# pnkraemer/experiments-lanczos-adjoints

Measured on AMD Instinct MI355X. Metric: slq_logdet_value_and_grad_throughput, higher is better.
Workload: dtype f32 (Gram contraction emulated with 3 f16 MFMA products, fp32 accumulate; accuracy vs fp64 at this size on 32 probe sets, profiles/r05b_accuracy_16_seeds/: value <= 5.6e-6 and d/d raw_noise <= 1.3e-5 on all 32; the other two gradient components <= 1e-4 on 25 of 32 sets, <= 1.5e-4 on 29, worst 3.96e-; 1 GPU; matrix-free RBF GP kernel N=131072 d=8, SLQ log-det value+grad, 40 Lanczos steps (full reortho) x 64 probes, fp32 (BASELINE config 4); N=131072, d=8, krylov_depth=40, probes_total=64, probes_on_this_rank=64, rows_on_this_rank=131072, gram_precision=f16x3, kernel=rbf

## Files before the change

experiments-lanczos-adjoints_amd/csrc/mfx_rbf.h:

```cpp
#pragma once
#include <type_traits>

#include "mfx_internal.h"

namespace mfx {

constexpr int kRbfMaxD = 1024;
inline int rbf_dpad(int d) { return d <= 4 ? 4 : d <= 8 ? 8 : d <= 12 ? 12 : d <= 16 ? 16 : d <= kRbfMaxD ? (d + 31) / 32 * 32 : -1; }

template <int V>
using Const = std::integral_constant<int, V>;

template <typename Narrow, typename WideFn>
static void with_dpad(int dpad, Narrow&& narrow, WideFn&& wide) {
  switch (dpad) {
    case 4: narrow(Const<4>{}); break;
    case 8: narrow(Const<8>{}); break;
    case 12: narrow(Const<12>{}); break;
    case 16: narrow(Const<16>{}); break;
    case 32: narrow(Const<32>{}); break;
    default: wide(); break;
  }
}

template <int MAXD, typename Launch>
static int with_mfma_dpad(int dpad, const char* not_built, Launch&& launch) {
  int rc = MFX_ERR_UNSUPPORTED;
  auto arm = [&](auto dc) {
    if constexpr (decltype(dc)::value <= MAXD) rc = launch(dc);
    else set_error("%s", not_built);
  };
  with_dpad(dpad, arm, [&] {
    if (dpad == 64) arm(Const<64>{});
    else if (dpad == 96) arm(Const<96>{});
    else if (dpad == 128) arm(Const<128>{});
    else set_error("%s", not_built);
  });
  return rc;
}

template <typename F>
static auto with_bool(bool flag, F&& f) {
  return flag ? f(std::true_type{}) : f(std::false_type{});
}
template <typename F>
static int with_kind(int kernel_fn, F&& f) {
  switch (kernel_fn) {
    case MFX_KERNEL_RBF: return f(Const<MFX_KERNEL_RBF>{});
    case MFX_KERNEL_MATERN12: return f(Const<MFX_KERNEL_MATERN12>{});
    case MFX_KERNEL_MATERN32: return f(Const<MFX_KERNEL_MATERN32>{});
    case MFX_KERNEL_MATERN52: return f(Const<MFX_KERNEL_MATERN52>{});
    default: set_error("unknown kernel_fn %d", kernel_fn); return MFX_ERR_INVALID;
  }
}

inline bool vec4_ok(const void* a, int64_t lda, const void* b, int64_t ldb, int64_t n, int64_t nrow) {
  return (n % 4 == 0) && (nrow % 4 == 0) && (lda % 4 == 0) && (ldb % 4 == 0) && (reinterpret_cast<uintptr_t>(a) % 16 == 0) &&
         (reinterpret_cast<uintptr_t>(b) % 16 == 0);
}

enum class RbfApplyPath { valu, exact, h3 };
enum class RbfGradPath { valu, exact, split };
RbfApplyPath rbf_apply_path(const mfx_operator* op, int64_t p);
RbfGradPath rbf_grad_path(const mfx_operator* op, int64_t batch, bool have_hws);

constexpr int64_t kRbfVscaleFloats = 65536 * 3;
constexpr int64_t kRbfVscaleMaxP = (kRbfVscaleFloats - 64) / 4;
static_assert(kRbfVscaleMaxP == 49136, "the limit the error message of the split matvec states");
struct RbfVscaleLayout {
  int64_t scales, amax_bits, rangeflag, amax_part;
  int64_t gx;
  bool ok;
};
RbfVscaleLayout rbf_vscale_layout(int64_t n, int64_t p);

struct RbfPackLayout {
  int64_t P, chunks, ntile;
  int64_t off_a, off_part;
  int nsplit;
  int64_t ldpart, bytes;
};
RbfPackLayout rbf_pack_layout(int64_t n, int64_t nrow, int64_t p, int dpad);
int64_t rbf_pack_ws_bytes(const mfx_operator* op, int64_t p);

struct RbfGradHLayout {
  int64_t bpad, npad, npad_l;
  int64_t amaxL, amaxR, scl, tail, perm, Lh, Ll, Rh, Rl, bytes;
};
RbfGradHLayout rbf_grad_h_layout(int64_t n, int64_t nrow, int64_t batch);
inline int64_t rbf_grad_h_ws_bytes(int64_t n, int64_t batch) { return rbf_grad_h_layout(n, n, batch).bytes; }

int64_t rbf_mfma_grad_partial_rows(int64_t n);

int rbf_mfma_apply(const mfx_operator* op, const float* xs, const float* sq, int dpad, const float* x, int64_t ldx,
                   float* y, int64_t ldy, int64_t p, hipStream_t stream);
int rbf_mfma_apply_h3(const mfx_operator* op, const float* xs, const float* sq, int dpad, const float* x, int64_t ldx,
                      float* y, int64_t ldy, int64_t p, float* vscale, void* pk, hipStream_t stream);
int rbf_mfma_grad(const mfx_operator* op, const float* xs, const float* sq, int dpad, const float* L, int64_t ldl,
                  const float* R, int64_t ldr, int64_t batch, double* partial, int64_t* nblocks_out,
                  hipStream_t stream);
int rbf_mfma_grad_h(const mfx_operator* op, const float* xs, const float* sq, int dpad, const float* L, int64_t ldl,
                    const float* R, int64_t ldr, int64_t batch, int64_t inner, double* partial, int64_t* nblocks_out, void* hws,
                    const float** scales_out, hipStream_t stream);

struct RbfMatvecArgs {
  const float *xs, *sq;
  int64_t n;
  const float *outputscale, *noise, *vscale, *x;
  int64_t ldx;
  float* y;
  int64_t ldy, p;
  const void *pkv, *pka;
  float* part;
  const int* rangeflag;
  int64_t ldpart, row0, rend;
};
int rbf_fat_launch(int dpad, int nb, bool vec4, dim3 grid, hipStream_t stream, const RbfMatvecArgs& a);

}
```

experiments-lanczos-adjoints_amd/csrc/mfx_rbf_fat.hip:

```cpp
#include <type_traits>

#include "mfx_internal.h"
#include "mfx_rbf_common.h"

namespace mfx {

struct FatSplit {
  int e[16], h[8], m[16];
};
constexpr FatSplit kFatSplit2 = {{0, 1, 2, 3, 4, 5, 5, 6, 7, 8, 9, 10, 10, 11, 12, 13},
                                 {2, 4, 6, 7, 9, 11, 12, 14},
                                 {3, 4, 5, 6, 7, 8, 8, 9, 10, 11, 12, 13, 13, 14, 15, 16}};
constexpr FatSplit kFatSplit1 = {{0, 0, 1, 1, 2, 2, 3, 3, 4, 4, 5, 5, 6, 6, 7, 7},
                                 {1, 2, 3, 4, 5, 6, 7, 8},
                                 {2, 3, 3, 4, 4, 5, 5, 6, 6, 7, 7, 8, 8, 9, 9, 10}};
template <int NB, int NKD>
struct FatPlan;
template <>
struct FatPlan<2, 2> {
  static constexpr int kSlots = 14;
  static constexpr FatSplit kSplit = kFatSplit2;
  static constexpr int dist_q(int slot) { return slot == 10 ? 0 : (slot == 12 ? 1 : -1); }
  static constexpr int contr_m(int slot) { return slot < 10 ? slot : (slot == 11 ? 10 : (slot == 13 ? 11 : -1)); }
  static constexpr int slot_of(int m) { return m < 10 ? m : (m == 10 ? 11 : 13); }
// ... 166 lines not shown
      }
    }
  };
  auto split_slot = [&](const int slot, const int lag, floatx16& w, half8 (&ah)[2], half8 (&al)[2], unsigned (&lopk)[8], const bool neg) {
#pragma unroll
    for (int i = 0; i < 16; ++i)
      if (Plan::kSplit.e[i] == slot + kSlots * lag) split_op(w, ah, al, lopk, 0, i, neg);
#pragma unroll
    for (int i = 0; i < 8; ++i)
      if (Plan::kSplit.h[i] == slot + kSlots * lag) split_op(w, ah, al, lopk, 1, i, neg);
#pragma unroll
    for (int i = 0; i < 16; ++i)
      if (Plan::kSplit.m[i] == slot + kSlots * lag) split_op(w, ah, al, lopk, 2, i, neg);
  };

  __builtin_amdgcn_s_waitcnt(0x0F70);
  __builtin_amdgcn_s_barrier();
  asm volatile("" ::: "memory");

  constexpr bool kRing4 = NB == 1;
  floatx16 wr[kRing4 ? 4 : 3];
#define MFX_WC(blk) wr[kRing4 ? ((blk) & 3) : 0]
#define MFX_WN(blk) wr[kRing4 ? (((blk) + 1) & 3) : 1]
#define MFX_WD(blk) wr[kRing4 ? (((blk) + 2) & 3) : 2]
  half8 ahc[2], alc[2], ahn[2], aln[2];
  unsigned lpc[8], lpn[8];
  half8 vf[2][NB][2];
  half8 ajs[2][NKD];
  read_a(ajs[0], 0, 0);
#pragma unroll
  for (int s = 0; s < 2; ++s)
#pragma unroll
    for (int nb = 0; nb < NB; ++nb)
#pragma unroll
      for (int hl = 0; hl < 2; ++hl) read_v1(vf[s][nb][hl], 0, 0, s, nb, hl);
#pragma unroll
  for (int q = 0; q < NKD; ++q) dist_step(MFX_WC(0), ajs[0][q], bih[0][q], q == 0);
#pragma unroll
  for (int q = 0; q < NKD; ++q) dist_step(MFX_WN(0), ajs[0][q], bih[1][q], q == 0);
  asm volatile("" : "+v"(MFX_WC(0)));
#pragma unroll
  for (int slot = 0; slot < kSlots; ++slot) split_slot(slot, 0, MFX_WC(0), ahc, alc, lpc, false);

  const float sc = outputscale[0];
  int tl = 0;
  for (; tl < ntl; ++tl) {
    const int buf = tl & 1;
    if (tl > 0 && (tl % kChainTiles) == 0) {
#pragma unroll
      for (int mi = 0; mi < 4; ++mi)
#pragma unroll
        for (int nb = 0; nb < NB; ++nb)
#pragma unroll
          for (int r = 0; r < 16; ++r) {
            mst[mi][nb][r] += acc[mi][nb][r];
            acc[mi][nb][r] = 0.f;
          }
    }
#pragma unroll
    for (int blk = 0; blk < 8; ++blk) {
      const int jb = blk >> 2, mi = blk & 3;
      const int blk1 = (blk + 1) & 7, blk2 = (blk + 2) & 7;
      const int jb2 = blk2 >> 2, mi2 = blk2 & 3;
      const bool neg_c = ((jb + mi) & 1) != 0, neg_n = (((blk1 >> 2) + (blk1 & 3)) & 1) != 0;
      if (blk == 5 && tl + 2 < ntl) issue_tile_dma(tl + 2);
#pragma unroll
      for (int slot = 0; slot < kSlots; ++slot) {
        __builtin_amdgcn_sched_barrier(0);
        if (Plan::dist_q(slot) >= 0) {
          const int q = Plan::dist_q(slot);
          dist_step(MFX_WD(blk), ajs[jb2 & 1][q], bih[mi2][q], q == 0);
        } else {
          const int m = Plan::contr_m(slot);
          const int s = m / (3 * NB), nb = (m / 3) % NB, w = m % 3;
          acc[mi][nb] = __builtin_amdgcn_mfma_f32_32x32x16_f16(w == 2 ? alc[s] : ahc[s], w == 1 ? vf[s][nb][1] : vf[s][nb][0],
                                                               acc[mi][nb], 0, 0, 0);
        }
        __builtin_amdgcn_sched_barrier(0);
        split_slot(slot, 1, MFX_WC(blk), ahc, alc, lpc, neg_c);
        split_slot(slot, 0, MFX_WN(blk), ahn, aln, lpn, neg_n);
        if (mi == 1 && slot < NKD) {
          ajs[(jb + 1) & 1][slot] = *reinterpret_cast<const half8*>(reinterpret_cast<const _Float16*>(fat_smem + (jb == 1 ? buf ^ 1 : buf) * S::kTile) +
                                                                   (((jb + 1) & 1) * 32 + l31) * AROW + slot * 16 + lhi * 8);
        }
        if (mi == 3) {
#pragma unroll
          for (int s = 0; s < 2; ++s)
#pragma unroll
            for (int nb = 0; nb < NB; ++nb)
#pragma unroll
              for (int hl = 0; hl < 2; ++hl) {
                const int mlast = 3 * NB * s + 3 * nb + (hl ? 1 : 2);
                if (Plan::slot_of(mlast) == slot) read_v1(vf[s][nb][hl], jb == 1 ? buf ^ 1 : buf, (jb + 1) & 1, s, nb, hl);
              }
        }
      }
      __builtin_amdgcn_sched_barrier(0);
      if (blk == 4) {
        __builtin_amdgcn_s_waitcnt(0x0F70);
        __builtin_amdgcn_s_barrier();
        asm volatile("" ::: "memory");
      }
      ahc[0] = ahn[0]; ahc[1] = ahn[1];
      alc[0] = aln[0]; alc[1] = aln[1];
      if constexpr (!kRing4) {
        wr[0] = wr[1];
        wr[1] = wr[2];
      }
#pragma unroll
      for (int q = 0; q < 8; ++q) lpc[q] = lpn[q];
    }
  }
  __builtin_amdgcn_s_waitcnt(0x0F70);
#pragma unroll
  for (int mi = 0; mi < 4; ++mi)
#pragma unroll
    for (int nb = 0; nb < NB; ++nb)
#pragma unroll
      for (int r = 0; r < 16; ++r) acc[mi][nb][r] += mst[mi][nb][r];
  const float nz = gridDim.z > 1 ? 0.f : noise[0];
  float* yout = gridDim.z > 1 ? part + (int64_t)blockIdx.z * p * ldpart : y;
  const int64_t ldo = gridDim.z > 1 ? ldpart : ldy;
#pragma unroll
  for (int mi = 0; mi < 4; ++mi)
#pragma unroll
    for (int nb = 0; nb < NB; ++nb) {
      const int64_t b = b0 + nb * 32 + l31;
      if (b >= p) continue;
      const float sb = sc * vscale[2 * b + 1] * (1.f / 32768.f);
#pragma unroll
      for (int g = 0; g < 4; ++g) {
        const int64_t i = i_wave + mi * 32 + 8 * g + 4 * lhi;
        if (VEC4 && i + 3 < rend) {
          const float4 xv = *reinterpret_cast<const float4*>(x + b * ldx + i);
          float4 o;
          o.x = fmaf(sb, acc[mi][nb][4 * g + 0], nz * xv.x);
          o.y = fmaf(sb, acc[mi][nb][4 * g + 1], nz * xv.y);
          o.z = fmaf(sb, acc[mi][nb][4 * g + 2], nz * xv.z);
          o.w = fmaf(sb, acc[mi][nb][4 * g + 3], nz * xv.w);
          *reinterpret_cast<float4*>(yout + b * ldo + (i - row0)) = o;
        } else {
#pragma unroll
          for (int e = 0; e < 4; ++e)
            if (i + e < rend) yout[b * ldo + (i - row0) + e] = fmaf(sb, acc[mi][nb][4 * g + e], nz * x[b * ldx + i + e]);
        }
      }
    }
}

#undef MFX_WC
#undef MFX_WN
#undef MFX_WD

int rbf_fat_launch(int dpad, int nb, bool vec4, dim3 grid, hipStream_t stream, const RbfMatvecArgs& a) {
  const char* not_built = "fat-wave Gram matvec supports d <= 16 and chunks of 32 or 64 vectors";
  MFX_REQUIRE(nb == 1 || nb == 2, MFX_ERR_UNSUPPORTED, "%s", not_built);
  return with_mfma_dpad<16>(dpad, not_built, [&](auto dc) -> int {
    return with_bool(nb == 2, [&](auto two) -> int {
      return with_bool(vec4, [&](auto v4) -> int {
        constexpr int DPAD = decltype(dc)::value, NB = decltype(two)::value ? 2 : 1;
        k_rbf_fat_apply<DPAD, decltype(v4)::value, NB><<<grid, 256, FatSmem<DPAD, NB>::kTotal, stream>>>(
            a.xs, a.sq, a.n, a.outputscale, a.noise, a.vscale, a.x, a.ldx, a.y, a.ldy, a.p, static_cast<const uintx4*>(a.pkv),
            static_cast<const uintx4*>(a.pka), a.part, a.rangeflag, a.ldpart, a.row0, a.rend);
        MFX_CHECK_LAUNCH();
        return MFX_OK;
      });
    });
  });
}

}
```

experiments-lanczos-adjoints_amd/csrc/mfx_rbf_mfma.hip:

```cpp
#include <stdlib.h>

#include <type_traits>

#include "mfx_internal.h"
#include "mfx_rbf_common.h"

namespace mfx {

constexpr int kGM = 128, kGN = 128, kGK = 32, kGSplit = 8;
constexpr int kGSub = 8;
constexpr int kGLd = kGM + 4;


__device__ __forceinline__ float dist_factor(int kind) {
  return kind == MFX_KERNEL_RBF ? -0.72134752044448170368f
                                : (kind == MFX_KERNEL_MATERN52 ? 5.f : (kind == MFX_KERNEL_MATERN32 ? 3.f : 1.f)) * kLog2e * kLog2e;
}

template <bool M52>
__device__ __forceinline__ void grad_weights(int kind, float dist, float& kv, float& wl) {
  if constexpr (M52) {
    const float r = __builtin_amdgcn_sqrtf(5.f * dist + kEpsF32);
    const float e = __builtin_amdgcn_exp2f(-kLog2e * r);
    kv = fmaf(r, fmaf(r, 1.f / 3.f, 1.f), 1.f) * e;
// ... 701 lines not shown
      }
#pragma unroll
      for (int m = NM1; m < NM; ++m) {
        __builtin_amdgcn_sched_barrier(0);
        contraction(m);
        __builtin_amdgcn_sched_barrier(0);
        if (has_next) {
#pragma unroll
          for (int pr = 0; pr < 8; ++pr)
            if (pr >= 8 * (m - NM1) / (NM - NM1) && pr < 8 * (m - NM1 + 1) / (NM - NM1))
              exp_split_pair(kdn, pr, kDiag && jbn == min_, negn, ahn, aln);
        }
      }
      __builtin_amdgcn_sched_barrier(0);
      if (has_next) {
        ah[0] = ahn[0]; ah[1] = ahn[1];
        al[0] = aln[0]; al[1] = aln[1];
      }
    }
    };
    if (KIND != MFX_KERNEL_RBF && t * kTJ == i_wave) {
      do_tile(std::true_type{});
    } else {
      do_tile(std::false_type{});
    }
    if (t + 1 < ntile) {
      if constexpr (!PK) store_tile(tile[(t + 1) & 1]);
    }
    __syncthreads();
  }
  if constexpr (PK) {
#pragma unroll
    for (int mi = 0; mi < kMI; ++mi)
#pragma unroll
      for (int nb = 0; nb < NB; ++nb) {
        const int idx = mi * NB + nb;
#pragma unroll
        for (int r = 0; r < 16; ++r) acc[mi][nb][r] += idx < kBlocks - 1 ? master[(idx * 16 + r) * 64] : mreg[r];
      }
  }
  const float s = outputscale[0], nz = gridDim.z > 1 ? 0.f : noise[0];
  float* yout = gridDim.z > 1 ? part + (int64_t)blockIdx.z * p * ldpart : y;
  const int64_t ldo = gridDim.z > 1 ? ldpart : ldy;
#pragma unroll
  for (int mi = 0; mi < kMI; ++mi)
#pragma unroll
    for (int nb = 0; nb < NB; ++nb) {
      const int64_t b = b0 + nb * 32 + l31;
      if (b >= p) continue;
      const float sb = s * vscale[2 * b + 1] * (1.f / 32768.f);
#pragma unroll
      for (int g = 0; g < 4; ++g) {
        const int64_t i = i_wave + mi * 32 + 8 * g + 4 * lhi;
        if (VEC4 && i + 3 < rend) {
          const float4 xv = *reinterpret_cast<const float4*>(x + b * ldx + i);
          float4 o;
          o.x = fmaf(sb, acc[mi][nb][4 * g + 0], nz * xv.x);
          o.y = fmaf(sb, acc[mi][nb][4 * g + 1], nz * xv.y);
          o.z = fmaf(sb, acc[mi][nb][4 * g + 2], nz * xv.z);
          o.w = fmaf(sb, acc[mi][nb][4 * g + 3], nz * xv.w);
          *reinterpret_cast<float4*>(yout + b * ldo + (i - row0)) = o;
        } else {
#pragma unroll
          for (int e = 0; e < 4; ++e)
            if (i + e < rend) yout[b * ldo + (i - row0) + e] = fmaf(sb, acc[mi][nb][4 * g + e], nz * x[b * ldx + i + e]);
        }
      }
    }
}

__global__ __launch_bounds__(256) void k_split_reduce(const float* __restrict__ part, int64_t ldpart, int nsplit, int64_t p,
                                                      int64_t nrow, int64_t ldy, const float* __restrict__ noise,
                                                      const float* __restrict__ x, int64_t ldx, float* __restrict__ y,
                                                      int64_t row0) {
  const int64_t i = (int64_t)blockIdx.x * 256 + threadIdx.x, b = blockIdx.y;
  if (i >= nrow) return;
  float acc = 0.f;
  for (int z = 0; z < nsplit; ++z) acc += part[((int64_t)z * p + b) * ldpart + i];
  y[b * ldy + i] = fmaf(noise[0], x[b * ldx + row0 + i], acc);
}

template <int DPAD, int NB, int KIND>
__global__ __launch_bounds__(256) void k_pack_tiles(const float* __restrict__ xs, const float* __restrict__ sq, int64_t n,
                                                    float* __restrict__ vscale, const float* __restrict__ amax_part, int gx,
                                                    const float* __restrict__ x, int64_t ldx, int64_t p,
                                                    uintx4* __restrict__ pkv, uintx4* __restrict__ pka, int* __restrict__ rangeflag) {
  constexpr int kTJ = 64;
  using Tile = RbfTileH3<DPAD, NB, kTJ>;
  constexpr int KD = Tile::KD, P = Tile::P, AROW = Tile::AROW;
  constexpr float cfac = KIND == MFX_KERNEL_RBF ? kNegHalfLog2e : matern_nu2<KIND>() * kLog2e * kLog2e;
  const int tid = threadIdx.x;
  const int64_t t = blockIdx.x, j0 = t * kTJ, ntile = gridDim.x;
  if ((int)blockIdx.y < (int)gridDim.y - 1) {
    const int64_t b0 = (int64_t)blockIdx.y * P;
    uintx4* dst = pkv + ((int64_t)blockIdx.y * ntile + t) * (2 * 8 * P);
    __shared__ float svs[P];
    if (tid < P) {
      const int64_t b = b0 + tid;
      float sc = 0.f;
      if (b < p) {
        float m = 0.f;
        for (int g = 0; g < gx; ++g) m = fmaxf(m, amax_part[b * gx + g]);
        sc = row_scale_of(m);
        if (t == 0) {
          vscale[2 * b] = sc;
          vscale[2 * b + 1] = 1.f / sc;
        }
      }
      svs[tid] = sc;
    }
    __syncthreads();
    for (int f0 = tid; f0 < 8 * P; f0 += 256) {
      const int row = f0 & 7, bq = f0 >> 3, f = row * P + bq;
      const int jb = row >> 2, s = (row >> 1) & 1, h = row & 1;
      const int64_t b = b0 + bq;
      half8 hh, ll;
      const float vs = svs[bq];
#pragma unroll
      for (int e = 0; e < 8; ++e) {
        const int64_t j = j0 + 32 * jb + 16 * s + 8 * (e >> 2) + 4 * h + (e & 3);
        const float v = (b < p && j < n) ? x[b * ldx + j] * vs : 0.f;
        float fh, fl;
        split_hi_lo(v, fh, fl);
        hh[e] = (_Float16)fh;
        ll[e] = (_Float16)fl;
      }
      dst[f] = __builtin_bit_cast(uintx4, hh);
      dst[8 * P + f] = __builtin_bit_cast(uintx4, ll);
    }
  } else {
    __shared__ __attribute__((aligned(16))) _Float16 img[kTJ][AROW];
    for (int e = tid; e < kTJ * AROW; e += 256) (&img[0][0])[e] = (_Float16)0.f;
    __syncthreads();
    for (int e = tid; e < kTJ * KD; e += 256) {
      const int j = e / KD, kk = e % KD;
      const int64_t jg = j0 + j;
      float v;
      if (kk < DPAD) v = jg < n ? -2.f * cfac * xs[jg * DPAD + kk] : 0.f;
      else if (kk == DPAD) v = cfac * (jg < n ? sq[jg] : 0.f) + (KIND == MFX_KERNEL_RBF ? kKShift : kEpsC);
      else v = cfac;
      if (fabsf(v) > 6.0e4f || (kk == DPAD && jg < n && sq[jg] > 6.0e4f)) atomicOr(rangeflag, 1);
      float hi, lo;
      split_hi_lo(((j >> 5) & 1) ? -v : v, hi, lo);
      img[j][kk] = (_Float16)hi;
      img[j][KD + kk] = (_Float16)hi;
      img[j][2 * KD + kk] = (_Float16)lo;
    }
    __syncthreads();
    uintx4* dst = pka + t * (kTJ * AROW * 2 / 16);
    for (int f = tid; f < kTJ * AROW * 2 / 16; f += 256) dst[f] = reinterpret_cast<const uintx4*>(&img[0][0])[f];
  }
}

static bool rbf_fat() {
  static const int v = [] {
    const char* e = getenv("MFX_RBF_FAT");
    return e ? atoi(e) : 1;
  }();
  return v != 0;
}

static int64_t chunk_width(int64_t p, int dpad) { return (p <= 32 || dpad > 16) ? 32 : 64; }

static int rbf_split_count(int64_t nrow, int64_t n, int64_t p, int dpad) {
  static const int forced = [] {
    const char* e = getenv("MFX_RBF_SPLIT");
    return e ? atoi(e) : 0;
  }();
  const int64_t pw = chunk_width(p, dpad);
  const int64_t wgs = ((nrow + 511) / 512) * ((p + pw - 1) / pw);
  const int64_t ntile = (n + 63) / 64;
  int64_t smax = ntile / 8;
  if (forced > 0) return forced <= 16 && forced <= ntile ? forced : 1;
  if (smax > 16) smax = 16;
  if (smax < 1 || wgs >= 2048) return 1;
  int best = 1;
  double best_cost = 1e30;
  for (int s = 1; s <= (int)smax; ++s) {
    const double rounds = (double)((wgs * s + 255) / 256);
    const double cost = rounds / s + 0.004 * s;
    if (cost < best_cost - 1e-12) {
      best_cost = cost;
      best = s;
    }
  }
  return best;
}

RbfPackLayout rbf_pack_layout(int64_t n, int64_t nrow, int64_t p, int dpad) {
  RbfPackLayout k;
  k.P = chunk_width(p, dpad);
  k.chunks = (p + k.P - 1) / k.P;
  k.ntile = (n + 63) / 64;
  const int64_t arow = ((3 * (dpad + 2) + 15) / 16) * 16 + 8;
  k.off_a = align_up(k.chunks * k.ntile * 2 * 8 * k.P * 16, 256);
  k.off_part = k.off_a + align_up(k.ntile * 64 * arow * 2, 256);
  k.nsplit = rbf_split_count(nrow, n, p, dpad);
  k.ldpart = align_up(nrow, 4);
  k.bytes = k.off_part + align_up((int64_t)k.nsplit * p * k.ldpart * 4, 256);
  return k;
}
int64_t rbf_pack_ws_bytes(const mfx_operator* op, int64_t p) {
  if (op->dtype != MFX_F32 || op->d > 32 || p < 1) return 0;
  return rbf_pack_layout(op->n, op_nrows(op), p, rbf_dpad(op->d)).bytes;
}

template <int DPAD, int NB, int KIND, bool PK>
static int launch_h3(bool vec4, dim3 grid, hipStream_t stream, const RbfMatvecArgs& a) {
  return with_bool(vec4, [&](auto v4) -> int {
    constexpr size_t kSm = 2 * sizeof(RbfTileH3<DPAD, NB, 64, !PK>) + (PK ? (size_t)8 * (2 * NB - 1) * 16 * 64 * 4 : 0);
    const auto kernel = k_rbf_mfma_apply_h3<DPAD, NB, decltype(v4)::value, KIND, PK, PK>;
    MFX_TRY(allow_big_lds(kernel, kSm));
    kernel<<<grid, 64 * H3Waves<PK>::value, kSm, stream>>>(a.xs, a.sq, a.n, a.outputscale, a.noise, a.vscale, a.x, a.ldx, a.y, a.ldy, a.p,
                                                           static_cast<const uintx4*>(a.pkv), static_cast<const uintx4*>(a.pka), a.part,
                                                           a.rangeflag, a.ldpart, a.row0, a.rend);
    return MFX_OK;
  });
}

template <int DPAD, int NB, int KIND>
static int launch_apply_h3k(const mfx_operator* op, const float* xs, const float* sq, const float* x, int64_t ldx,
                            float* y, int64_t ldy, int64_t p, float* vscale, void* pk, hipStream_t stream) {
  const int64_t n = op->n;
  const int64_t row0 = op_row0(op), nrow = op_nrows(op), rend = row0 + nrow;
  MFX_REQUIRE(row0 % 64 == 0, MFX_ERR_INVALID, "matrix-core Gram matvec: row0 = %lld must be a multiple of 64", (long long)row0);
  constexpr bool kPackBuilt = DPAD <= 16 || NB == 1;
  const bool pack = pk != nullptr && kPackBuilt;
  const RbfVscaleLayout vl = rbf_vscale_layout(n, p);
  MFX_REQUIRE(vl.ok, MFX_ERR_UNSUPPORTED, "matrix-core Gram matvec: %lld vectors exceed the scale / slice-maximum region of the workspace (at most %lld)", (long long)p, (long long)kRbfVscaleMaxP);
  int* rangeflag = reinterpret_cast<int*>(vscale + vl.rangeflag);
  float* amax_part = vscale + vl.amax_part;
  if (pack) {
    k_row_amax_part<<<dim3((unsigned)vl.gx, (unsigned)p), 256, 0, stream>>>(x, ldx, n, amax_part, rangeflag);
    MFX_CHECK_LAUNCH();
  } else {
    MFX_TRY(row_scales(x, ldx, n, p, vscale, vl, stream));
  }
  const unsigned chunks = (unsigned)((p + NB * 32 - 1) / (NB * 32));
  const bool vec4 = vec4_ok(x, ldx, y, ldy, n, nrow);
  const RbfPackLayout pl = rbf_pack_layout(n, nrow, p, DPAD);
  char* pkb = static_cast<char*>(pk);
  const int nsplit = pk ? pl.nsplit : 1;
  RbfMatvecArgs a{xs, sq, n, (const float*)op->outputscale, (const float*)op->noise, vscale, x, ldx, y, ldy, p, nullptr, nullptr,
                  pk ? reinterpret_cast<float*>(pkb + pl.off_part) : nullptr, nullptr, pl.ldpart, row0, rend};
  const dim3 grid((unsigned)((nrow + 255) / 256), chunks, (unsigned)nsplit);
  const dim3 grid_pk((unsigned)((nrow + 511) / 512), chunks, (unsigned)nsplit);
  if constexpr (kPackBuilt) {
    if (pack) {
      a.pkv = pkb;
      a.pka = pkb + pl.off_a;
      a.rangeflag = rangeflag;
      k_pack_tiles<DPAD, NB, KIND><<<dim3((unsigned)pl.ntile, chunks + 1), 256, 0, stream>>>(
          xs, sq, n, vscale, amax_part, (int)vl.gx, x, ldx, p, static_cast<uintx4*>(pk), reinterpret_cast<uintx4*>(pkb + pl.off_a), rangeflag);
      MFX_CHECK_LAUNCH();
      bool fat = false;
      if constexpr (KIND == MFX_KERNEL_RBF && DPAD <= 16) fat = rbf_fat();
      if (fat) MFX_TRY(rbf_fat_launch(DPAD, NB, vec4, grid_pk, stream, a));
      else MFX_TRY((launch_h3<DPAD, NB, KIND, true>(vec4, grid_pk, stream, a)));
    }
  }
  MFX_TRY((launch_h3<DPAD, NB, KIND, false>(vec4, grid, stream, a)));
  MFX_CHECK_LAUNCH();
  if (nsplit > 1) {
    k_split_reduce<<<dim3((unsigned)((nrow + 255) / 256), (unsigned)p), 256, 0, stream>>>(a.part, a.ldpart, nsplit, p, nrow, ldy,
                                                                                        (const float*)op->noise, x, ldx, y, row0);
    MFX_CHECK_LAUNCH();
  }
  return MFX_OK;
}

int rbf_mfma_apply_h3(const mfx_operator* op, const float* xs, const float* sq, int dpad, const float* x, int64_t ldx,
                      float* y, int64_t ldy, int64_t p, float* vscale, void* pk, hipStream_t stream) {
  const bool two_blocks = pk ? chunk_width(p, dpad) == 64 : p > 32;
  return with_mfma_dpad<32>(dpad, "split matrix-core Gram matvec supports d <= 32", [&](auto dc) -> int {
    return with_bool(two_blocks, [&](auto two) -> int {
      return with_kind(op->kernel_fn, [&](auto kind) -> int {
        return launch_apply_h3k<decltype(dc)::value, decltype(two)::value ? 2 : 1, decltype(kind)::value>(op, xs, sq, x, ldx, y, ldy, p,
                                                                                                         vscale, pk, stream);
      });
    });
  });
}

__global__ __launch_bounds__(256) void k_row_amax(const float* __restrict__ x, int64_t ldx, int64_t n,
                                                  float* __restrict__ amax) {
  __shared__ float sm[4];
  const int64_t b = blockIdx.x;
  float m = 0.f;
  for (int64_t i = threadIdx.x; i < n; i += 256) m = fmaxf(m, fabsf(x[b * ldx + i]));
#pragma unroll
  for (int o = 32; o > 0; o >>= 1) m = fmaxf(m, __shfl_xor(m, o, 64));
  if ((threadIdx.x & 63) == 0) sm[threadIdx.x >> 6] = m;
  __syncthreads();
  if (threadIdx.x == 0) amax[b] = fmaxf(fmaxf(sm[0], sm[1]), fmaxf(sm[2], sm[3]));
}

__global__ void k_global_scale(const float* __restrict__ amax, int64_t rows, float* __restrict__ scale) {
  __shared__ float sm[256];
  float m = 0.f;
  for (int64_t i = threadIdx.x; i < rows; i += 256) m = fmaxf(m, amax[i]);
  sm[threadIdx.x] = m;
  __syncthreads();
  for (int o = 128; o > 0; o >>= 1) {
    if ((int)threadIdx.x < o) sm[threadIdx.x] = fmaxf(sm[threadIdx.x], sm[threadIdx.x + o]);
    __syncthreads();
  }
  if (threadIdx.x == 0) {
    int e = 0;
    float s = 1.f;
    if (sm[0] > 0.f && sm[0] < 3.0e38f) {
      frexpf(sm[0], &e);
      s = ldexpf(1.f, 14 - e < 126 ? 14 - e : 126);
    }
    scale[0] = s;
    scale[1] = 1.f / s;
  }
}

__host__ __device__ __forceinline__ bool grad_col_sign(int64_t i, uint32_t salt) {
  uint32_t h = (uint32_t)i * 0x9E3779B1u + salt;
  h ^= h >> 15;
  h *= 0x85EBCA77u;
  h ^= h >> 13;
  h *= 0xC2B2AE3Du;
  return (h >> 31) != 0;
}
constexpr uint32_t kSaltL = 0x51ED270Bu, kSaltR = 0xB5297A4Du;

#ifndef MFX_GRAD_ONE_PRODUCT_LOG2
#define MFX_GRAD_ONE_PRODUCT_LOG2 10
#endif
static int grad_one_product_log2() {
  static const int v = [] {
    const char* e = getenv("MFX_GRAD_ONE_PRODUCT_LOG2");
    const int x = e ? atoi(e) : MFX_GRAD_ONE_PRODUCT_LOG2;
    return x < 0 ? 0 : (x > 60 ? 60 : x);
  }();
  return v;
}
constexpr int kSortMax = 8192;
__global__ __launch_bounds__(1024) void k_order_rows(const float* __restrict__ amaxL, const float* __restrict__ amaxR, int64_t batch,
                                                     int64_t inner, int64_t bpad, int npow2, int one_log2, int* __restrict__ perm,
                                                     int* __restrict__ tail) {
  extern __shared__ unsigned long long keys[];
  const int64_t outer = batch / inner;
  for (int i = threadIdx.x; i < npow2; i += 1024) {
    unsigned long long kv = 0;
    if (i < batch) {
      const int64_t src = inner > 1 ? ((int64_t)i % outer) * inner + (int64_t)i / outer : i;
      float m = amaxL[src] * amaxR[src];
      if (!(m >= 0.f) || m > 3.0e38f) m = 3.0e38f;
      kv = ((unsigned long long)__float_as_uint(m) << 32) | (unsigned long long)(0xFFFFFFFFu - (unsigned)i);
    }
    keys[i] = kv;
  }
  __syncthreads();
  for (int size = 2; size <= npow2; size <<= 1)
    for (int stride = size >> 1; stride > 0; stride >>= 1) {
      for (int t = threadIdx.x; t < npow2 / 2; t += 1024) {
        const int lo = 2 * t - (t & (stride - 1)), hi = lo + stride;
        const bool desc = (lo & size) == 0;
        const unsigned long long a = keys[lo], b = keys[hi];
        if (desc ? a < b : a > b) {
          keys[lo] = b;
          keys[hi] = a;
        }
      }
      __syncthreads();
    }
  for (int64_t bt = threadIdx.x; bt < bpad; bt += 1024) {
    int src = -1;
    if (bt < batch) {
      const int64_t i = 0xFFFFFFFFu - (unsigned)(keys[bt] & 0xFFFFFFFFull);
      src = (int)(inner > 1 ? (i % outer) * inner + i / outer : i);
    }
    perm[bt] = src;
  }
  __shared__ double wave_sum[16];
  __shared__ int first_row;
  const int nstage = (int)(bpad / 32);
  if (one_log2 <= 0) {
    if (threadIdx.x == 0) tail[0] = nstage;
    return;
  }
  const int per = npow2 >= 1024 ? npow2 / 1024 : 1;
  const int64_t r0 = (int64_t)threadIdx.x * per, r1 = r0 + per < batch ? r0 + per : batch;
  double mine = 0.0;
  for (int64_t bt = r1 - 1; bt >= r0; --bt) mine += (double)__uint_as_float((unsigned)(keys[bt] >> 32));
  const int lane = threadIdx.x & 63, wv = threadIdx.x >> 6;
  double suf = mine;
#pragma unroll
  for (int off = 1; off < 64; off <<= 1) {
    const double o = __shfl_down(suf, off, 64);
    if (lane + off < 64) suf += o;
  }
  if (lane == 0) wave_sum[wv] = suf;
  if (threadIdx.x == 0) first_row = (int)batch;
  __syncthreads();
  double behind = 0.0, total = 0.0;
  for (int w = 0; w < 16; ++w) {
    total += wave_sum[w];
    if (w > wv) behind += wave_sum[w];
  }
  const double cut = total < 1.0e38 ? ldexp(total, -one_log2) : -1.0;
  double mass = behind + (suf - mine);
  int64_t first = r1;
  for (int64_t bt = r1 - 1; bt >= r0; --bt) {
    const double m = (double)__uint_as_float((unsigned)(keys[bt] >> 32));
    if (mass + m > cut) break;
    mass += m;
// ... 748 lines not shown
```

Measured before the change: 94.74 probes/s.

## Add fat-wave Gram matvec variant using 16x16x32 MFMA for d<=8

Adds a new fat-wave split-f16 Gram matvec kernel for d<=8 with 64-vector chunks. It computes the distance product as a single 16x16x32 f16 MFMA k-step, interleaves the exp2/hi-lo split chain with the contraction MFMAs through a slot table, and double-buffers tile DMA into shared memory. It becomes the default through a new MFX_RBF_FAT mode value of 2. The aim is to cut MFMA count and idle time in the hot Lanczos matvec, at the cost of a large hand-scheduled kernel that relies on s_nop hazard padding and AGPR hints.

```diff
diff --git a/experiments-lanczos-adjoints_amd/csrc/mfx_rbf.h b/experiments-lanczos-adjoints_amd/csrc/mfx_rbf.h
--- a/experiments-lanczos-adjoints_amd/csrc/mfx_rbf.h
+++ b/experiments-lanczos-adjoints_amd/csrc/mfx_rbf.h
@@ -115,6 +115,6 @@
   const int* rangeflag;
   int64_t ldpart, row0, rend;
 };
-int rbf_fat_launch(int dpad, int nb, bool vec4, dim3 grid, hipStream_t stream, const RbfMatvecArgs& a);
+int rbf_fat_launch(int dpad, int nb, bool vec4, bool wide16, dim3 grid, hipStream_t stream, const RbfMatvecArgs& a);
 
 }
diff --git a/experiments-lanczos-adjoints_amd/csrc/mfx_rbf_fat.hip b/experiments-lanczos-adjoints_amd/csrc/mfx_rbf_fat.hip
--- a/experiments-lanczos-adjoints_amd/csrc/mfx_rbf_fat.hip
+++ b/experiments-lanczos-adjoints_amd/csrc/mfx_rbf_fat.hip
@@ -342,9 +342,259 @@
 #undef MFX_WN
 #undef MFX_WD
 
-int rbf_fat_launch(int dpad, int nb, bool vec4, dim3 grid, hipStream_t stream, const RbfMatvecArgs& a) {
+struct Fat16Tab {
+  int e[8], h[4], m[8];
+};
+constexpr Fat16Tab kFat16Tab = {{0, 1, 2, 3, 4, 5, 6, 7}, {8, 8, 9, 9}, {10, 11, 10, 11, 12, 13, 12, 13}};
+
+template <int DPAD, bool VEC4>
+__global__ __launch_bounds__(256, 1) void k_rbf_fat_apply16(const float* __restrict__ xs, const float* __restrict__ sq, int64_t n,
+                                                            const float* __restrict__ outputscale, const float* __restrict__ noise,
+                                                            const float* __restrict__ vscale, const float* __restrict__ x,
+                                                            int64_t ldx, float* __restrict__ y, int64_t ldy, int64_t p,
+                                                            const uintx4* __restrict__ pkv, const uintx4* __restrict__ pka,
+                                                            float* __restrict__ part, const int* __restrict__ rangeflag,
+                                                            int64_t ldpart, int64_t row0, int64_t rend) {
+  if (rangeflag && *rangeflag != 0) return;
+  using S = FatSmem<DPAD, 2>;
+  constexpr int KD = S::KD, AROW = S::AROW;
+  static_assert(S::NKD == 2 && 3 * KD <= 32, "the distance product is one k-step of 32");
+  constexpr Fat16Tab T = kFat16Tab;
+  extern __shared__ __attribute__((aligned(16))) char fat_smem[];
+  const int tid = threadIdx.x, lane = tid & 63;
+  const int wid = __builtin_amdgcn_readfirstlane(tid >> 6);
+  const int l15 = lane & 15, lg = lane >> 4;
+  const int64_t i_wave = row0 + (int64_t)blockIdx.x * 512 + wid * 128;
+  const int64_t b0 = (int64_t)blockIdx.y * 64;
+  const int64_t ntile_all = (n + 63) / 64;
+  const int64_t t_first = ntile_all * blockIdx.z / gridDim.z;
+  const int ntl = (int)(ntile_all * (blockIdx.z + 1) / gridDim.z - t_first);
+
+  float agpr_seed = 0.f;
+  asm volatile("; accumulators in AGPRs" : "+a"(agpr_seed));
+
+  auto issue_tile_dma = [&](int tl) {
+    const char* asrc = reinterpret_cast<const char*>(pka) + (t_first + tl) * (int64_t)S::kABytes;
+    const char* vsrc = reinterpret_cast<const char*>(pkv) + ((int64_t)blockIdx.y * ntile_all + t_first + tl) * S::kVBytes;
+    char* dst = fat_smem + (tl & 1) * S::kTile;
+#pragma unroll
+    for (int c = 0; c < (S::kABytes / 1024 + 3) / 4; ++c) {
+      const int piece = wid + 4 * c;
+      if (piece < S::kABytes / 1024) glds16(asrc + piece * 1024 + lane * 16, dst + piece * 1024);
+    }
+#pragma unroll
+    for (int c = 0; c < S::kVBytes / 4096; ++c) glds16(vsrc + (wid + 4 * c) * 1024 + lane * 16, dst + S::kABytes + (wid + 4 * c) * 1024);
+  };
+  if (0 < ntl) issue_tile_dma(0);
+  if (1 < ntl) issue_tile_dma(1);
+
+  half8 bi[8];
+#pragma unroll
+  for (int it = 0; it < 8; ++it) {
+    int64_t i = i_wave + it * 16 + l15;
+    if (i >= rend) i = rend - 1;
+    if (i < row0) i = row0;
+#pragma unroll
+    for (int e = 0; e < 8; ++e) {
+      const int slot = lg * 8 + e;
+      const int comp = slot / KD, kk = slot % KD;
+      float v = 0.f;
+      if (comp < 3) v = (kk < DPAD) ? xs[i * DPAD + kk] : (kk == DPAD ? 1.f : sq[i]);
+      float hi, lo;
+      split_hi_lo(v, hi, lo);
+      const float w = comp == 1 ? lo : hi;
+      bi[it][e] = (_Float16)(((it >> 1) & 1) ? -w : w);
+    }
+  }
+  floatx4 acc[8][4], mst[8][4];
+#pragma unroll
+  for (int it = 0; it < 8; ++it)
+#pragma unroll
+    for (int pg = 0; pg < 4; ++pg)
+#pragma unroll
+      for (int r = 0; r < 4; ++r) {
+        acc[it][pg][r] = 0.f;
+        mst[it][pg][r] = 0.f;
+      }
+  acc[0][0][0] = agpr_seed;
+
+  auto read_a = [&](half8& a, int buf, int jb, int c2) {
+    const _Float16* img = reinterpret_cast<const _Float16*>(fat_smem + buf * S::kTile);
+    a = *reinterpret_cast<const half8*>(img + (jb * 32 + 16 * (l15 >> 3) + 8 * c2 + (l15 & 7)) * AROW + lg * 8);
+  };
+  auto read_v = [&](half8& v, int buf, int jb, int f) {
+    v = *reinterpret_cast<const half8*>(fat_smem + buf * S::kTile + S::kABytes + (f & 1) * (8 * S::kVRow) + (jb * 4 + lg) * S::kVRow +
+                                        ((f >> 1) * 16 + l15) * 16);
+  };
+  auto dist16 = [&](floatx4& kd, const half8& a, const half8& b) {
+    asm volatile("s_nop 1\n\tv_mfma_f32_16x16x32_f16 %0, %1, %2, 0" : "=&v"(kd) : "v"(a), "v"(b));
+  };
+  auto chain = [&](floatx4 (&w)[2], half8& ah, half8& al, unsigned (&lp)[4], const int t, const int i, const bool neg) {
+    if (t == 0) {
+      w[i >> 2][i & 3] = __builtin_amdgcn_exp2f(neg ? -w[i >> 2][i & 3] : w[i >> 2][i & 3]);
+    } else if (t == 1) {
+      const half2v h = {(_Float16)w[i >> 1][(2 * i) & 3], (_Float16)w[i >> 1][(2 * i + 1) & 3]};
+      ah[2 * i] = h[0];
+      ah[2 * i + 1] = h[1];
+    } else {
+      const int pr = i >> 1;
+      const half2v h = {ah[2 * pr], ah[2 * pr + 1]};
+      const unsigned hb = __builtin_bit_cast(unsigned, h);
+      if ((i & 1) == 0) {
+        asm("v_fma_mixlo_f16 %0, %1, -1.0, %2 op_sel:[0,0,0] op_sel_hi:[1,0,0]" : "=v"(lp[pr]) : "v"(hb), "v"(w[i >> 2][i & 3]));
+      } else {
+        asm("v_fma_mixhi_f16 %0, %1, -1.0, %2 op_sel:[1,0,0] op_sel_hi:[1,0,0]" : "+v"(lp[pr]) : "v"(hb), "v"(w[i >> 2][i & 3]));
+        const half2v l = __builtin_bit_cast(half2v, lp[pr]);
+        al[2 * pr] = l[0];
+        al[2 * pr + 1] = l[1];
+      }
+    }
+  };
+  auto chain_slot = [&](const int slot, floatx4 (&w)[2], half8& ah, half8& al, unsigned (&lp)[4], const bool neg) {
+#pragma unroll
+    for (int i = 0; i < 8; ++i)
+      if (T.e[i] == slot) chain(w, ah, al, lp, 0, i, neg);
+#pragma unroll
+    for (int i = 0; i < 4; ++i)
+      if (T.h[i] == slot) chain(w, ah, al, lp, 1, i, neg);
+#pragma unroll
+    for (int i = 0; i < 8; ++i)
+      if (T.m[i] == slot) chain(w, ah, al, lp, 2, i, neg);
+  };
+
+  __builtin_amdgcn_s_waitcnt(0x0F70);
+  __builtin_amdgcn_s_barrier();
+  asm volatile("" ::: "memory");
+
+  floatx4 wr[4][2];
+  half8 ah[2], al[2];
+  unsigned lp[4];
+  half8 vf[2][8];
+  half8 aj[2][2];
+#pragma unroll
+  for (int c2 = 0; c2 < 2; ++c2) read_a(aj[0][c2], 0, 0, c2);
+#pragma unroll
+  for (int f = 0; f < 8; ++f) read_v(vf[0][f], 0, 0, f);
+#pragma unroll
+  for (int c2 = 0; c2 < 2; ++c2) dist16(wr[0][c2], aj[0][c2], bi[0]);
+#pragma unroll
+  for (int c2 = 0; c2 < 2; ++c2) dist16(wr[1][c2], aj[0][c2], bi[1]);
+  asm volatile("s_nop 15\n\ts_nop 15" : "+v"(wr[0][0]), "+v"(wr[0][1]), "+v"(wr[1][0]), "+v"(wr[1][1]));
+#pragma unroll
+  for (int slot = 0; slot < 14; ++slot) chain_slot(slot, wr[0], ah[0], al[0], lp, false);
+
+  const float sc = outputscale[0];
+  for (int tl = 0; tl < ntl; ++tl) {
+    const int buf = tl & 1;
+    if (tl > 0 && (tl % kChainTiles) == 0) {
+#pragma unroll
+      for (int it = 0; it < 8; ++it)
+#pragma unroll
+        for (int pg = 0; pg < 4; ++pg)
+#pragma unroll
+          for (int r = 0; r < 4; ++r) {
+            mst[it][pg][r] += acc[it][pg][r];
+            acc[it][pg][r] = 0.f;
+          }
+    }
+    auto unit = [&](auto uc) {
+      constexpr int u = decltype(uc)::value;
+      constexpr int jb = u >> 3, it = u & 7;
+      constexpr int u1 = (u + 1) & 15, u2 = (u + 2) & 15;
+      constexpr bool neg_n = (((u1 >> 3) + ((u1 & 7) >> 1)) & 1) != 0;
+      const int nbuf = jb == 1 ? buf ^ 1 : buf;
+      if (u == 9 && tl + 2 < ntl) issue_tile_dma(tl + 2);
+#pragma unroll
+      for (int slot = 0; slot < 14; ++slot) {
+        __builtin_amdgcn_sched_barrier(0);
+        if (slot == 8 || slot == 10) {
+          const int c2 = (slot - 8) / 2;
+          dist16(wr[(u + 2) & 3][c2], aj[(u2 >> 3) & 1][c2], bi[u2 & 7]);
+        } else {
+          const int m = slot < 8 ? slot : (slot == 9 ? 8 : slot - 2);
+          const int w = m / 4, pg = m % 4;
+          acc[it][pg] = __builtin_amdgcn_mfma_f32_16x16x32_f16(w == 2 ? al[u & 1] : ah[u & 1], w == 1 ? vf[jb][pg * 2 + 1] : vf[jb][pg * 2],
+                                                               acc[it][pg], 0, 0, 0);
+        }
+        __builtin_amdgcn_sched_barrier(0);
+        chain_slot(slot, wr[(u + 1) & 3], ah[(u + 1) & 1], al[(u + 1) & 1], lp, neg_n);
+        if (slot == 2) read_v(vf[jb ^ 1][it], nbuf, jb ^ 1, it);
+        if (it == 3 && (slot == 4 || slot == 5)) read_a(aj[jb ^ 1][slot - 4], nbuf, jb ^ 1, slot - 4);
+      }
+      __builtin_amdgcn_sched_barrier(0);
+      if (u == 7) {
+        __builtin_amdgcn_s_waitcnt(0x0070);
+        __builtin_amdgcn_s_barrier();
+        asm volatile("" ::: "memory");
+      }
+    };
+    unit(std::integral_constant<int, 0>{});
+    unit(std::integral_constant<int, 1>{});
+    unit(std::integral_constant<int, 2>{});
+    unit(std::integral_constant<int, 3>{});
+    unit(std::integral_constant<int, 4>{});
+    unit(std::integral_constant<int, 5>{});
+    unit(std::integral_constant<int, 6>{});
+    unit(std::integral_constant<int, 7>{});
+    unit(std::integral_constant<int, 8>{});
+    unit(std::integral_constant<int, 9>{});
+    unit(std::integral_constant<int, 10>{});
+    unit(std::integral_constant<int, 11>{});
+    unit(std::integral_constant<int, 12>{});
+    unit(std::integral_constant<int, 13>{});
+    unit(std::integral_constant<int, 14>{});
+    unit(std::integral_constant<int, 15>{});
+  }
+  __builtin_amdgcn_s_waitcnt(0x0F70);
+#pragma unroll
+  for (int it = 0; it < 8; ++it)
+#pragma unroll
+    for (int pg = 0; pg < 4; ++pg)
+#pragma unroll
+      for (int r = 0; r < 4; ++r) acc[it][pg][r] += mst[it][pg][r];
+  const float nz = gridDim.z > 1 ? 0.f : noise[0];
+  float* yout = gridDim.z > 1 ? part + (int64_t)blockIdx.z * p * ldpart : y;
+  const int64_t ldo = gridDim.z > 1 ? ldpart : ldy;
+#pragma unroll
+  for (int pg = 0; pg < 4; ++pg) {
+    const int64_t b = b0 + pg * 16 + l15;
+    if (b >= p) continue;
+    const float sb = sc * vscale[2 * b + 1] * (1.f / 32768.f);
+#pragma unroll
+    for (int it = 0; it < 8; ++it) {
+      const int64_t i = i_wave + it * 16 + 4 * lg;
+      if (VEC4 && i + 3 < rend) {
+        const float4 xv = *reinterpret_cast<const float4*>(x + b * ldx + i);
+        float4 o;
+        o.x = fmaf(sb, acc[it][pg][0], nz * xv.x);
+        o.y = fmaf(sb, acc[it][pg][1], nz * xv.y);
+        o.z = fmaf(sb, acc[it][pg][2], nz * xv.z);
+        o.w = fmaf(sb, acc[it][pg][3], nz * xv.w);
+        *reinterpret_cast<float4*>(yout + b * ldo + (i - row0)) = o;
+      } else {
+#pragma unroll
+        for (int e = 0; e < 4; ++e)
+          if (i + e < rend) yout[b * ldo + (i - row0) + e] = fmaf(sb, acc[it][pg][e], nz * x[b * ldx + i + e]);
+      }
+    }
+  }
+}
+
+int rbf_fat_launch(int dpad, int nb, bool vec4, bool wide16, dim3 grid, hipStream_t stream, const RbfMatvecArgs& a) {
   const char* not_built = "fat-wave Gram matvec supports d <= 16 and chunks of 32 or 64 vectors";
   MFX_REQUIRE(nb == 1 || nb == 2, MFX_ERR_UNSUPPORTED, "%s", not_built);
+  if (wide16 && nb == 2 && dpad <= 8) {
+    return with_mfma_dpad<8>(dpad, not_built, [&](auto dc) -> int {
+      return with_bool(vec4, [&](auto v4) -> int {
+        constexpr int DPAD = decltype(dc)::value;
+        k_rbf_fat_apply16<DPAD, decltype(v4)::value><<<grid, 256, FatSmem<DPAD, 2>::kTotal, stream>>>(
+            a.xs, a.sq, a.n, a.outputscale, a.noise, a.vscale, a.x, a.ldx, a.y, a.ldy, a.p, static_cast<const uintx4*>(a.pkv),
+            static_cast<const uintx4*>(a.pka), a.part, a.rangeflag, a.ldpart, a.row0, a.rend);
+        MFX_CHECK_LAUNCH();
+        return MFX_OK;
+      });
+    });
+  }
   return with_mfma_dpad<16>(dpad, not_built, [&](auto dc) -> int {
     return with_bool(nb == 2, [&](auto two) -> int {
       return with_bool(vec4, [&](auto v4) -> int {
diff --git a/experiments-lanczos-adjoints_amd/csrc/mfx_rbf_mfma.hip b/experiments-lanczos-adjoints_amd/csrc/mfx_rbf_mfma.hip
--- a/experiments-lanczos-adjoints_amd/csrc/mfx_rbf_mfma.hip
+++ b/experiments-lanczos-adjoints_amd/csrc/mfx_rbf_mfma.hip
@@ -877,12 +877,14 @@
   }
 }
 
-static bool rbf_fat() {
+constexpr int kRbfFatDefault = 2;
+static int rbf_fat() {
   static const int v = [] {
     const char* e = getenv("MFX_RBF_FAT");
-    return e ? atoi(e) : 1;
+    const int m = e ? atoi(e) : kRbfFatDefault;
+    return m == 0 || m == 1 ? m : 2;
   }();
-  return v != 0;
+  return v;
 }
 
 static int64_t chunk_width(int64_t p, int dpad) { return (p <= 32 || dpad > 16) ? 32 : 64; }
@@ -978,9 +980,9 @@
       k_pack_tiles<DPAD, NB, KIND><<<dim3((unsigned)pl.ntile, chunks + 1), 256, 0, stream>>>(
           xs, sq, n, vscale, amax_part, (int)vl.gx, x, ldx, p, static_cast<uintx4*>(pk), reinterpret_cast<uintx4*>(pkb + pl.off_a), rangeflag);
       MFX_CHECK_LAUNCH();
-      bool fat = false;
+      int fat = 0;
       if constexpr (KIND == MFX_KERNEL_RBF && DPAD <= 16) fat = rbf_fat();
-      if (fat) MFX_TRY(rbf_fat_launch(DPAD, NB, vec4, grid_pk, stream, a));
+      if (fat) MFX_TRY(rbf_fat_launch(DPAD, NB, vec4, fat == 2, grid_pk, stream, a));
       else MFX_TRY((launch_h3<DPAD, NB, KIND, true>(vec4, grid_pk, stream, a)));
     }
   }
```

Result: faster. 97.50 probes/s (median of 6 runs) (+2.9%).
